# linto-ai/whisper-timestamped

Hardware: NVIDIA H100
Metric: audio-sec/s (RTF) large-v3 1h synthetic @1/2/4/8 H100; DTW GB/s vs HBM peak (higher is better)
Workload: dtype bf16x3 tensor-core GEMMs (float32-accurate), f32 elsewhere, f64 DTW accumulate

## Files before the change

include/wts.h:

```cpp
#ifndef WTS_H
#define WTS_H

#include <stdint.h>

#ifdef __cplusplus
extern "C" {
#endif

#define WTS_VERSION 102
#define WTS_SEG_NONPOSITIVE 1
#define WTS_SEG_PITCH16 2

typedef struct WtsSegDesc {
    int32_t window;
    int32_t row0;
    int32_t last_row;
    int32_t T;
    int32_t f0;
    int32_t F;
    int32_t max_dur;
    int32_t flags;
    int64_t cost_off;
    int64_t jumps_off;
    int64_t dir_off;
// ... 18 lines not shown
int wts_dtw_batch(const void* d_cost, int32_t cost_is_f64,
                  const WtsSegDesc* d_segs, int32_t nseg,
                  uint32_t* d_dir_ws, double* d_bnd_ws,
                  int32_t* d_jumps, int32_t* d_path, const int64_t* d_path_off,
                  int32_t* d_path_len, int32_t* d_status, void* stream);

int wts_dtw_batch_sized(const void* d_cost, int32_t cost_is_f64,
                  const WtsSegDesc* d_segs, int32_t nseg,
                  uint32_t* d_dir_ws, double* d_bnd_ws,
                  int32_t* d_jumps, int32_t* d_path, const int64_t* d_path_off,
                  int32_t* d_path_len, int32_t* d_status, int32_t max_T, int32_t max_F, int32_t all_flags,
                  void* stream);

int wts_disfluency_starts(const float* d_cost, const WtsSegDesc* d_segs, int32_t nseg, const int32_t* d_jumps,
                          int32_t* d_out, void* stream);



typedef struct WtsGemm {
    const void* a;  int64_t lda, a_plane, a_bo, a_bi;
    const void* b;  int64_t ldb, b_plane, b_bo, b_bi;
    int32_t M, N, K, batch_outer, batch_inner;
    float alpha;
    const float* bias;
    int32_t bias_on_m;
    int32_t act;
    const float* residual; int64_t ldr, r_bo, r_bi;
    float* out_f32;   int64_t ldc, c_bo, c_bi;
    void*  out_sb16;  int64_t ldo, o_plane, o_bo, o_bi;
    int32_t head_dim; int64_t head_stride;
    int32_t backend;
    int32_t a_is_f32, b_is_f32;
    const int32_t* row_mask;
} WtsGemm;

int wts_gemm(const WtsGemm* g, void* stream);

int wts_to_sb16(const float* d_x, int64_t n, void* d_hi, void* d_lo, void* stream);

int wts_layernorm(const float* d_x, int64_t ldx, const float* d_gamma, const float* d_beta, int32_t M,
                  int32_t D, void* d_out_sb16, int64_t ldo, int64_t o_plane, float* d_out_f32, int64_t ldf,
                  void* stream);

int wts_softmax_rows(const float* d_s, int64_t lds, int64_t rows, int32_t n, void* d_out_sb16, int64_t ldo,
                     int64_t o_plane, void* stream);

int wts_enc_attention(const void* d_qk, int64_t ld_qk, int64_t qk_plane, const void* d_vt, int64_t ld_vt,
                      int64_t vt_plane, int32_t B, int32_t H, int32_t D, int32_t n_ctx, void* d_out, int64_t ldo,
                      int64_t o_plane, void* stream);

int wts_frames(const float* d_audio, int64_t n_samples, int64_t n_total, int64_t n_frames, void* d_out,
               int64_t o_plane, void* stream);
int wts_power(const float* d_y, int64_t ldy, int64_t n_frames, void* d_out, int64_t ldo, int64_t o_plane,
              void* stream);
int wts_logmel_max(const float* d_m, int64_t n, float* d_max, void* stream);
int wts_logmel_finish(const float* d_m, int64_t n_frames, int32_t n_mels, const float* d_max, float* d_out_f32,
                      void* stream);

int wts_window_gather(const int64_t* d_mel_ptr, int32_t n_mels, const int32_t* d_seek, const int32_t* d_size,
                      int32_t B, void* d_out, int64_t o_plane, void* stream);

int wts_embed(const int32_t* d_tokens, const int32_t* d_positions, const float* d_emb, const float* d_pos,
              int32_t rows, int32_t D, float* d_out, void* stream);

int wts_gather_rows(const float* d_x, int64_t ldx, const int32_t* d_idx, int32_t rows, int32_t D, float* d_out,
                    void* stream);
// ... 84 lines not shown
```

whisper-timestamped_b200/csrc/gemm_tc.cu:

```cuda
#include <cuda_bf16.h>

#include <stdlib.h>

#include "sm90.cuh"

namespace wts {

constexpr int BM = 128, BN = 128, BK = 64;
constexpr int TILE_BYTES = BM * BK * 2;
constexpr int STAGES = 3;
constexpr int STAGE_BYTES = 4 * TILE_BYTES;
constexpr int GT_THREADS = 288;
constexpr int PT_THREADS = 384;
constexpr int PT_PRODUCER_REGS = 40, PT_CONSUMER_REGS = 232;
static_assert(128 * PT_PRODUCER_REGS + 256 * PT_CONSUMER_REGS <= 65536, "setmaxnreg plan exceeds the register file");
constexpr int GROUP_M = 8;
constexpr int GT_SMEM = STAGES * STAGE_BYTES + 256 + 1024;
constexpr int PART_LD = BN + 4;
static_assert(BM * PART_LD * 4 <= STAGES * STAGE_BYTES, "the partial tile lives in the operand ring");

__device__ __forceinline__ float gelu_erf_tc(float v) { return 0.5f * v * (1.0f + erff(v * 0.70710678118654752440f)); }

struct TcArgs {
    WtsGemm g;
    int a_has_bo, a_has_bi, b_has_bo, b_has_bi;
    int split_k;
    int pair_stores;
};

__device__ __forceinline__ int64_t out_offset(const WtsGemm& g, int m, int n, int64_t ld)
{
    return g.head_dim > 0 ? (int64_t)(n / g.head_dim) * g.head_stride + (int64_t)m * ld + (n % g.head_dim)
                          : (int64_t)m * ld + n;
}

__device__ __forceinline__ void store_one(const WtsGemm& g, int m, int n, float t, float* of, __nv_bfloat16* ob)
{
    if (of) of[out_offset(g, m, n, g.ldc)] = t;
    if (ob) {
        const __nv_bfloat16 hi = __float2bfloat16_rn(t);
        __nv_bfloat16* d = ob + out_offset(g, m, n, g.ldo);
        d[0] = hi;
        d[g.o_plane] = __float2bfloat16_rn(t - __bfloat162float(hi));
    }
}

__device__ __forceinline__ float2 pair_values(const WtsGemm& g, int n, bool two, float v0, float v1, float bias_m, const float* res)
{
    float t0 = g.alpha * v0, t1 = g.alpha * v1;
    if (g.bias) {
        t0 += g.bias_on_m ? bias_m : g.bias[n];
        if (two) t1 += g.bias_on_m ? bias_m : g.bias[n + 1];
    }
    if (g.act == 1) { t0 = gelu_erf_tc(t0); t1 = gelu_erf_tc(t1); }
    if (res) { t0 += res[n]; if (two) t1 += res[n + 1]; }
    return make_float2(t0, t1);
}

__device__ __forceinline__ void store_pair_sb16(__nv_bfloat16* dh, int64_t plane, float t0, float t1)
{
// ... 174 lines not shown
            float v[64];
#pragma unroll
            for (int i = 0; i < 64; ++i) v[i] = h ? acc[1][i] : acc[0][i];
            if (pairs) epilogue_frag64<true>(g, tc.zo, tc.zi, tc.m0 + 64 * h + 16 * warp, tc.n0, v);
            else epilogue_frag64<false>(g, tc.zo, tc.zi, tc.m0 + 64 * h + 16 * warp, tc.n0, v);
        }
    }
}

__global__ void __launch_bounds__(GT_THREADS, 1)
gemm_tc_skinny_kernel(const __grid_constant__ CUtensorMap tmA, const __grid_constant__ CUtensorMap tmB, const TcArgs args)
{
    extern __shared__ unsigned char smem_raw[];
    const WtsGemm& g = args.g;
    const uint32_t base = (smem_addr(smem_raw) + 1023u) & ~1023u;
    const uint32_t bar = base + STAGES * STAGE_BYTES;
    const int warp = threadIdx.x >> 5, lane = threadIdx.x & 31;
    const int n0 = blockIdx.x * BN, m0 = blockIdx.y * BM;
    const int S = args.split_k;
    const int z = S > 1 ? 0 : blockIdx.z, zo = z / g.batch_inner, zi = z - zo * g.batch_inner;
    const int nkb_all = (g.K + BK - 1) / BK;
    const int part_k = S > 1 ? blockIdx.z : 0;
    const int kb0 = (int)((int64_t)part_k * nkb_all / S);
    const int nkb = (int)((int64_t)(part_k + 1) * nkb_all / S) - kb0;
    pdl_launch();

    if (threadIdx.x == 256) {
        asm volatile("prefetch.tensormap [%0];" ::"l"(&tmA) : "memory");
        asm volatile("prefetch.tensormap [%0];" ::"l"(&tmB) : "memory");
        for (int s = 0; s < STAGES; ++s) { mbar_init(bar + 8 * s, 1); mbar_init(bar + 32 + 8 * s, 8); }
        asm volatile("fence.mbarrier_init.release.cluster;" ::: "memory");
    }
    __syncthreads();
    pdl_wait();

    float acc[64];
    if (warp == 8) {
        if (lane == 0) {
            const int azo = args.a_has_bo ? zo : 0, azi = args.a_has_bi ? zi : 0;
            const int bzo = args.b_has_bo ? zo : 0, bzi = args.b_has_bi ? zi : 0;
            for (int kb = 0; kb < nkb; ++kb) {
                const int s = kb % STAGES, u = kb / STAGES;
                mbar_wait(bar + 32 + 8 * s, (u & 1) ^ 1);
                const uint32_t full = bar + 8 * s;
                mbar_expect_tx(full, STAGE_BYTES);
                const uint32_t st = base + s * STAGE_BYTES;
                const int kc = (kb0 + kb) * BK;
                tma_load_5d(st, &tmA, full, kc, m0, azi, azo, 0);
                tma_load_5d(st + TILE_BYTES, &tmA, full, kc, m0, azi, azo, 1);
                tma_load_5d(st + 2 * TILE_BYTES, &tmB, full, kc, n0, bzi, bzo, 0);
                tma_load_5d(st + 3 * TILE_BYTES, &tmB, full, kc, n0, bzi, bzo, 1);
            }
        }
    } else {
        const int wg = warp >> 2;
#pragma unroll
        for (int i = 0; i < 64; ++i) acc[i] = 0.f;
        for (int kb = 0; kb < nkb; ++kb) {
            const int s = kb % STAGES, u = kb / STAGES;
            mbar_wait(bar + 8 * s, u & 1);
            const uint32_t st = base + s * STAGE_BYTES;
            const uint64_t a_hi = wg_desc(st + wg * (TILE_BYTES / 2)), a_lo = wg_desc(st + TILE_BYTES + wg * (TILE_BYTES / 2));
            const uint64_t b_hi = wg_desc(st + 2 * TILE_BYTES), b_lo = wg_desc(st + 3 * TILE_BYTES);
            wg_fence();
#pragma unroll
            for (int k = 0; k < BK / 16; ++k) {
                const uint64_t adv = (uint64_t)(k * 2);
                wgmma_ss_n128(acc, a_hi + adv, b_hi + adv, 1);
                wgmma_ss_n128(acc, a_lo + adv, b_hi + adv, 1);
                wgmma_ss_n128(acc, a_hi + adv, b_lo + adv, 1);
            }
            wg_commit();
            wg_wait<1>();
            if (kb > 0 && lane == 0) mbar_arrive(bar + 32 + 8 * ((kb - 1) % STAGES));
        }
        wg_wait<0>();

        const int rl = 64 * wg + 16 * (warp & 3) + (lane >> 2);
        const int cl = 2 * (lane & 3);
        if (S == 1) {
            epilogue_frag64<false>(g, zo, zi, m0 + 64 * wg + 16 * (warp & 3), n0, acc);
        } else {
// ... 76 lines not shown
    }
    return 0;
}

int gemm_tc_launch(const WtsGemm& g, cudaStream_t st)
{
    static int n_sm = 0;
    if (n_sm == 0) {
        WTS_CUDA_CHECK(cudaFuncSetAttribute(gemm_tc_kernel, cudaFuncAttributeMaxDynamicSharedMemorySize, GT_SMEM));
        WTS_CUDA_CHECK(cudaFuncSetAttribute(gemm_tc_skinny_kernel, cudaFuncAttributeMaxDynamicSharedMemorySize, GT_SMEM));
        int dev = 0;
        WTS_CUDA_CHECK(cudaGetDevice(&dev));
        WTS_CUDA_CHECK(cudaDeviceGetAttribute(&n_sm, cudaDevAttrMultiProcessorCount, dev));
    }
    alignas(64) CUtensorMap tmA, tmB;
    int rc = make_map(&tmA, g.a, g.K, g.M, g.lda, g.a_plane, g.batch_inner, g.a_bi, g.batch_outer, g.a_bo, BM, "A");
    if (rc) return rc;
    rc = make_map(&tmB, g.b, g.K, g.N, g.ldb, g.b_plane, g.batch_inner, g.b_bi, g.batch_outer, g.b_bo, BN, "B");
    if (rc) return rc;
    TcArgs args;
    args.g = g;
    args.a_has_bo = g.a_bo != 0; args.a_has_bi = g.a_bi != 0;
    args.b_has_bo = g.b_bo != 0; args.b_has_bi = g.b_bi != 0;
    const int tiles_n = (g.N + BN - 1) / BN, tiles_m = (g.M + BM - 1) / BM, nkb = (g.K + BK - 1) / BK;
    const int batch = g.batch_outer * g.batch_inner;
    cudaLaunchConfig_t cfg = {};
    cfg.dynamicSmemBytes = GT_SMEM;
    cfg.stream = st;
    const bool skinny = tiles_m == 1 && batch == 1 && g.head_dim == 0;
    if (!skinny) {
        const int64_t tiles = (int64_t)tiles_m * tiles_n * batch;
        if (tiles > INT32_MAX / 2) { set_error("wts_gemm(tc): %lld output tiles are too many", (long long)tiles); return -7; }
        args.split_k = 1;
        const bool heads_even = g.head_dim == 0 || (g.head_dim % 2 == 0 && g.head_stride % 2 == 0);
        const bool of_pairs = !g.out_f32 || ((reinterpret_cast<uintptr_t>(g.out_f32) & 7) == 0 && g.ldc % 2 == 0 &&
                                             g.c_bo % 2 == 0 && g.c_bi % 2 == 0);
        const bool ob_pairs = !g.out_sb16 || ((reinterpret_cast<uintptr_t>(g.out_sb16) & 3) == 0 && g.ldo % 2 == 0 &&
                                              g.o_plane % 2 == 0 && g.o_bo % 2 == 0 && g.o_bi % 2 == 0);
        args.pair_stores = !g.row_mask && heads_even && of_pairs && ob_pairs;
        cfg.gridDim = dim3((unsigned)(tiles < n_sm ? tiles : n_sm), 1, 1);
        cfg.blockDim = dim3(PT_THREADS, 1, 1);
        WTS_CUDA_CHECK(cudaLaunchKernelEx(&cfg, gemm_tc_kernel, tmA, tmB, args));
        return 0;
    }
    static const int splitk = []{ const char* e = getenv("WTS_SPLITK"); return e ? atoi(e) : 1; }();
    int split = 1;
    if (splitk && 2 * tiles_n <= n_sm) {
        split = n_sm / tiles_n;
        if (split > 8) split = 8;
        if (split > nkb) split = nkb;
    }
    args.split_k = split;
    args.pair_stores = 0;
    cfg.gridDim = dim3(tiles_n, 1, split);
    cfg.blockDim = dim3(GT_THREADS, 1, 1);
    cudaLaunchAttribute attr[2];
    int na = 0;
    if (split > 1) {
        attr[na].id = cudaLaunchAttributeClusterDimension;
        attr[na].val.clusterDim.x = 1;
        attr[na].val.clusterDim.y = 1;
        attr[na].val.clusterDim.z = split;
        ++na;
    }
    if (pdl_enabled()) {
        attr[na].id = cudaLaunchAttributeProgrammaticStreamSerialization;
        attr[na].val.programmaticStreamSerializationAllowed = 1;
        ++na;
    }
    cfg.attrs = attr;
    cfg.numAttrs = na;
    WTS_CUDA_CHECK(cudaLaunchKernelEx(&cfg, gemm_tc_skinny_kernel, tmA, tmB, args));
    return 0;
}

}
```

whisper-timestamped_b200/csrc/ops.cu:

```cuda
#include "decode_common.cuh"

namespace wts {

__global__ void to_sb16_kernel(const float* __restrict__ x, int64_t n, __nv_bfloat16* __restrict__ hi,
                               __nv_bfloat16* __restrict__ lo)
{
    for (int64_t i = blockIdx.x * (int64_t)blockDim.x + threadIdx.x; i < n; i += (int64_t)gridDim.x * blockDim.x) {
        __nv_bfloat16 h, l;
        split_bf16(x[i], h, l);
        hi[i] = h;
        lo[i] = l;
    }
}

constexpr int LN_THREADS = 128, LN_MAXV = 16;
__global__ void __launch_bounds__(LN_THREADS)
layernorm_kernel(const float* x, int64_t ldx, const float* gamma,
                 const float* beta, int M, int D, __nv_bfloat16* o, int64_t ldo,
                 int64_t o_plane, float* of, int64_t ldf)
{
    pdl_launch();
    pdl_wait();
    __shared__ float red[32];
    const int row = blockIdx.x;
    const float* xr = x + (int64_t)row * ldx;
    float v[LN_MAXV];
    float s = 0.f;
#pragma unroll
    for (int k = 0; k < LN_MAXV; ++k) {
        const int c = threadIdx.x + LN_THREADS * k;
        v[k] = c < D ? xr[c] : 0.f;
        s += v[k];
    }
    const float mean = block_reduce_sum(s, red) / (float)D;
    float q = 0.f;
#pragma unroll
    for (int k = 0; k < LN_MAXV; ++k) {
        const int c = threadIdx.x + LN_THREADS * k;
        const float d = c < D ? v[k] - mean : 0.f;
        q += d * d;
    }
    const float rstd = 1.0f / sqrtf(block_reduce_sum(q, red) / (float)D + 1e-5f);
#pragma unroll
    for (int k = 0; k < LN_MAXV; ++k) {
        const int c = threadIdx.x + LN_THREADS * k;
        if (c < D) {
            const float y = (v[k] - mean) * rstd * gamma[c] + beta[c];
            if (o) {
                __nv_bfloat16 h, l;
                split_bf16(y, h, l);
                o[(int64_t)row * ldo + c] = h;
                o[(int64_t)row * ldo + c + o_plane] = l;
            }
            if (of) of[(int64_t)row * ldf + c] = y;
        }
    }
}

__global__ void __launch_bounds__(128)
softmax_rows_kernel(const float* __restrict__ s, int64_t lds, int64_t rows, int n,
                    __nv_bfloat16* __restrict__ o, int64_t ldo, int64_t o_plane)
{
    const int64_t row = (int64_t)blockIdx.x * 4 + (threadIdx.x >> 5);
    const int lane = threadIdx.x & 31;
    if (row >= rows) return;
    const float* sr = s + row * lds;
    float v[64];
    float mx = -CUDART_INF_F;
#pragma unroll
    for (int k = 0; k < 64; ++k) {
        const int c = lane + 32 * k;
        v[k] = c < n ? sr[c] : -CUDART_INF_F;
        mx = fmaxf(mx, v[k]);
    }
    mx = warp_max(mx);
    float sum = 0.f;
#pragma unroll
    for (int k = 0; k < 64; ++k) {
        v[k] = expf(v[k] - mx);
        sum += v[k];
// ... 324 lines not shown
    float mx = -CUDART_INF_F;
    for (int v = threadIdx.x; v < n; v += blockDim.x) mx = fmaxf(mx, x[v]);
    mx = block_reduce_max(mx, red);
    float s = 0.f;
    for (int v = threadIdx.x; v < n; v += blockDim.x) s += expf(x[v] - mx);
    s = block_reduce_sum(s, red);
    if (threadIdx.x == 0) out[blockIdx.x] = (x[tokens[blockIdx.x]] - mx) - logf(s);
}

}

using namespace wts;

static inline int grid_for(int64_t n, int block, int cap = 132 * 16)
{
    int64_t g = (n + block - 1) / block;
    return (int)(g < 1 ? 1 : (g > cap ? cap : g));
}

extern "C" int wts_to_sb16(const float* d_x, int64_t n, void* d_hi, void* d_lo, void* stream)
{
    if (n <= 0) return 0;
    to_sb16_kernel<<<grid_for(n, 256), 256, 0, (cudaStream_t)stream>>>(d_x, n, (__nv_bfloat16*)d_hi, (__nv_bfloat16*)d_lo);
    WTS_LAUNCH_CHECK();
    return 0;
}

extern "C" int wts_layernorm(const float* d_x, int64_t ldx, const float* d_gamma, const float* d_beta, int32_t M,
                             int32_t D, void* d_out_sb16, int64_t ldo, int64_t o_plane, float* d_out_f32,
                             int64_t ldf, void* stream)
{
    if (M <= 0) return 0;
    if (D > LN_THREADS * LN_MAXV) { set_error("wts_layernorm: D=%d > %d", D, LN_THREADS * LN_MAXV); return -2; }
    WTS_CUDA_CHECK(launch_pdl(layernorm_kernel, dim3(M), dim3(LN_THREADS), 0, (cudaStream_t)stream, d_x, ldx, d_gamma, d_beta, M, D,
                                                                   (__nv_bfloat16*)d_out_sb16, ldo, o_plane, d_out_f32, ldf));
    WTS_LAUNCH_CHECK();
    return 0;
}

extern "C" int wts_softmax_rows(const float* d_s, int64_t lds, int64_t rows, int32_t n, void* d_out_sb16,
                                int64_t ldo, int64_t o_plane, void* stream)
{
    if (rows <= 0) return 0;
    if (n > 2048) { set_error("wts_softmax_rows: n=%d > 2048", n); return -2; }
    softmax_rows_kernel<<<(unsigned)((rows + 3) / 4), 128, 0, (cudaStream_t)stream>>>(d_s, lds, rows, n,
                                                                                     (__nv_bfloat16*)d_out_sb16, ldo, o_plane);
    WTS_LAUNCH_CHECK();
    return 0;
}

extern "C" int wts_frames(const float* d_audio, int64_t n_samples, int64_t n_total, int64_t n_frames, void* d_out,
                          int64_t o_plane, void* stream)
{
    (void)o_plane;
    if (n_frames <= 0) return 0;
    frames_kernel<<<(unsigned)n_frames, 128, 0, (cudaStream_t)stream>>>(d_audio, n_samples, n_total, n_frames, (float*)d_out);
    WTS_LAUNCH_CHECK();
    return 0;
}

extern "C" int wts_power(const float* d_y, int64_t ldy, int64_t n_frames, void* d_out, int64_t ldo, int64_t o_plane,
                         void* stream)
{
    (void)o_plane;
    if (n_frames <= 0) return 0;
    power_kernel<<<(unsigned)((n_frames * 208 + 255) / 256), 256, 0, (cudaStream_t)stream>>>(d_y, ldy, n_frames, (float*)d_out, ldo);
    WTS_LAUNCH_CHECK();
// ... 179 lines not shown
```

whisper-timestamped_b200/csrc/sm90.cuh:

```cuda
#pragma once
#include <cuda.h>
#include <cudaTypedefs.h>

#include <mutex>

#include "common.cuh"

namespace wts {

__device__ __forceinline__ uint32_t smem_addr(const void* p) { return (uint32_t)__cvta_generic_to_shared(p); }

__device__ __forceinline__ void mbar_init(uint32_t bar, uint32_t count)
{
    asm volatile("mbarrier.init.shared::cta.b64 [%0], %1;" ::"r"(bar), "r"(count));
}
__device__ __forceinline__ void mbar_expect_tx(uint32_t bar, uint32_t bytes)
{
    asm volatile("mbarrier.arrive.expect_tx.shared::cta.b64 _, [%0], %1;" ::"r"(bar), "r"(bytes) : "memory");
}
__device__ __forceinline__ void mbar_arrive(uint32_t bar)
{
    asm volatile("mbarrier.arrive.shared::cta.b64 _, [%0];" ::"r"(bar) : "memory");
}
__device__ __forceinline__ void mbar_wait(uint32_t bar, uint32_t parity)
{
    asm volatile(
        "{\n\t"
        ".reg .pred p;\n\t"
        "WAIT_LOOP:\n\t"
        "mbarrier.try_wait.parity.shared::cta.b64 p, [%0], %1;\n\t"
        "@p bra DONE;\n\t"
        "bra WAIT_LOOP;\n\t"
        "DONE:\n\t"
        "}\n" ::"r"(bar), "r"(parity) : "memory");
}
__device__ __forceinline__ void tma_load_4d(uint32_t dst, const CUtensorMap* tm, uint32_t bar, int c0, int c1, int c2, int c3)
{
    asm volatile(
        "cp.async.bulk.tensor.4d.shared::cluster.global.mbarrier::complete_tx::bytes [%0], [%1, {%3, %4, %5, %6}], [%2];"
        ::"r"(dst), "l"(tm), "r"(bar), "r"(c0), "r"(c1), "r"(c2), "r"(c3) : "memory");
}
__device__ __forceinline__ void tma_load_5d(uint32_t dst, const CUtensorMap* tm, uint32_t bar, int c0, int c1, int c2,
                                            int c3, int c4)
{
    asm volatile(
        "cp.async.bulk.tensor.5d.shared::cluster.global.mbarrier::complete_tx::bytes [%0], [%1, {%3, %4, %5, %6, %7}], [%2];"
        ::"r"(dst), "l"(tm), "r"(bar), "r"(c0), "r"(c1), "r"(c2), "r"(c3), "r"(c4) : "memory");
}

__device__ __forceinline__ uint64_t wg_desc(uint32_t saddr)
{
    uint64_t d = 0;
    d |= (uint64_t)((saddr >> 4) & 0x3FFF);
    d |= (uint64_t)1 << 16;
    d |= (uint64_t)(1024 >> 4) << 32;
    d |= (uint64_t)1 << 62;
    return d;
}
__device__ __forceinline__ void wg_fence() { asm volatile("wgmma.fence.sync.aligned;" ::: "memory"); }
__device__ __forceinline__ void wg_commit() { asm volatile("wgmma.commit_group.sync.aligned;" ::: "memory"); }
template <int N> __device__ __forceinline__ void wg_wait() { asm volatile("wgmma.wait_group.sync.aligned %0;" ::"n"(N) : "memory"); }

__device__ __forceinline__ void wgmma_ss_n128(float (&d)[64], uint64_t a, uint64_t b, int scale_d)
{
    asm volatile(
        "{\n\t.reg .pred p;\n\tsetp.ne.b32 p, %66, 0;\n\t"
        "wgmma.mma_async.sync.aligned.m64n128k16.f32.bf16.bf16 {%0, %1, %2, %3, %4, %5, %6, %7, %8, %9, %10, %11, %12, %13, %14, %15, %16, %17, %18, %19, %20, %21, %22, %23, %24, %25, %26, %27, %28, %29, %30, %31, %32, %33, %34, %35, %36, %37, %38, %39, %40, %41, %42, %43, %44, %45, %46, %47, %48, %49, %50, %51, %52, %53, %54, %55, %56, %57, %58, %59, %60, %61, %62, %63}, %64, %65, p, 1, 1, 0, 0;\n\t}\n"
        : "+f"(d[0]), "+f"(d[1]), "+f"(d[2]), "+f"(d[3]), "+f"(d[4]), "+f"(d[5]), "+f"(d[6]), "+f"(d[7]), "+f"(d[8]), "+f"(d[9]), "+f"(d[10]), "+f"(d[11]), "+f"(d[12]), "+f"(d[13]), "+f"(d[14]), "+f"(d[15]), "+f"(d[16]), "+f"(d[17]), "+f"(d[18]), "+f"(d[19]), "+f"(d[20]), "+f"(d[21]), "+f"(d[22]), "+f"(d[23]), "+f"(d[24]), "+f"(d[25]), "+f"(d[26]), "+f"(d[27]), "+f"(d[28]), "+f"(d[29]), "+f"(d[30]), "+f"(d[31]), "+f"(d[32]), "+f"(d[33]), "+f"(d[34]), "+f"(d[35]), "+f"(d[36]), "+f"(d[37]), "+f"(d[38]), "+f"(d[39]), "+f"(d[40]), "+f"(d[41]), "+f"(d[42]), "+f"(d[43]), "+f"(d[44]), "+f"(d[45]), "+f"(d[46]), "+f"(d[47]), "+f"(d[48]), "+f"(d[49]), "+f"(d[50]), "+f"(d[51]), "+f"(d[52]), "+f"(d[53]), "+f"(d[54]), "+f"(d[55]), "+f"(d[56]), "+f"(d[57]), "+f"(d[58]), "+f"(d[59]), "+f"(d[60]), "+f"(d[61]), "+f"(d[62]), "+f"(d[63])
        : "l"(a), "l"(b), "r"(scale_d));
}

__device__ __forceinline__ void wgmma_rs_n64(float (&d)[32], const uint32_t* a, uint64_t b)
{
    asm volatile(
        "{\n\t.reg .pred p;\n\tsetp.ne.b32 p, %37, 0;\n\t"
        "wgmma.mma_async.sync.aligned.m64n64k16.f32.bf16.bf16 {%0, %1, %2, %3, %4, %5, %6, %7, %8, %9, %10, %11, %12, %13, %14, %15, %16, %17, %18, %19, %20, %21, %22, %23, %24, %25, %26, %27, %28, %29, %30, %31}, {%32, %33, %34, %35}, %36, p, 1, 1, 0;\n\t}\n"
        : "+f"(d[0]), "+f"(d[1]), "+f"(d[2]), "+f"(d[3]), "+f"(d[4]), "+f"(d[5]), "+f"(d[6]), "+f"(d[7]), "+f"(d[8]), "+f"(d[9]), "+f"(d[10]), "+f"(d[11]), "+f"(d[12]), "+f"(d[13]), "+f"(d[14]), "+f"(d[15]), "+f"(d[16]), "+f"(d[17]), "+f"(d[18]), "+f"(d[19]), "+f"(d[20]), "+f"(d[21]), "+f"(d[22]), "+f"(d[23]), "+f"(d[24]), "+f"(d[25]), "+f"(d[26]), "+f"(d[27]), "+f"(d[28]), "+f"(d[29]), "+f"(d[30]), "+f"(d[31])
        : "r"(a[0]), "r"(a[1]), "r"(a[2]), "r"(a[3]), "l"(b), "r"(1));
}

// ... 22 lines not shown
```

whisper-timestamped_b200/whisper_timestamped/_native.py:

```python
import ctypes
import os

import numpy as np
import torch

_HERE = os.path.dirname(os.path.abspath(__file__))
LIB_PATH = os.path.join(_HERE, "libwts.so")


class WtsError(RuntimeError):
    pass


class SegDesc(ctypes.Structure):
    _fields_ = [
        ("window", ctypes.c_int32), ("row0", ctypes.c_int32), ("last_row", ctypes.c_int32),
        ("T", ctypes.c_int32), ("f0", ctypes.c_int32), ("F", ctypes.c_int32),
        ("max_dur", ctypes.c_int32), ("flags", ctypes.c_int32),
        ("cost_off", ctypes.c_int64), ("jumps_off", ctypes.c_int64),
        ("dir_off", ctypes.c_int64), ("bnd_off", ctypes.c_int64),
    ]


SEG_DTYPE = np.dtype([
    ("window", "<i4"), ("row0", "<i4"), ("last_row", "<i4"), ("T", "<i4"), ("f0", "<i4"),
    ("F", "<i4"), ("max_dur", "<i4"), ("flags", "<i4"), ("cost_off", "<i8"), ("jumps_off", "<i8"),
    ("dir_off", "<i8"), ("bnd_off", "<i8")])
assert SEG_DTYPE.itemsize == ctypes.sizeof(SegDesc) == 64


class Gemm(ctypes.Structure):
    _fields_ = [
        ("a", ctypes.c_void_p), ("lda", ctypes.c_int64), ("a_plane", ctypes.c_int64), ("a_bo", ctypes.c_int64), ("a_bi", ctypes.c_int64),
        ("b", ctypes.c_void_p), ("ldb", ctypes.c_int64), ("b_plane", ctypes.c_int64), ("b_bo", ctypes.c_int64), ("b_bi", ctypes.c_int64),
        ("M", ctypes.c_int32), ("N", ctypes.c_int32), ("K", ctypes.c_int32), ("batch_outer", ctypes.c_int32), ("batch_inner", ctypes.c_int32),
        ("alpha", ctypes.c_float),
        ("bias", ctypes.c_void_p), ("bias_on_m", ctypes.c_int32), ("act", ctypes.c_int32),
        ("residual", ctypes.c_void_p), ("ldr", ctypes.c_int64), ("r_bo", ctypes.c_int64), ("r_bi", ctypes.c_int64),
        ("out_f32", ctypes.c_void_p), ("ldc", ctypes.c_int64), ("c_bo", ctypes.c_int64), ("c_bi", ctypes.c_int64),
        ("out_sb16", ctypes.c_void_p), ("ldo", ctypes.c_int64), ("o_plane", ctypes.c_int64), ("o_bo", ctypes.c_int64), ("o_bi", ctypes.c_int64),
        ("head_dim", ctypes.c_int32), ("head_stride", ctypes.c_int64),
        ("backend", ctypes.c_int32), ("a_is_f32", ctypes.c_int32), ("b_is_f32", ctypes.c_int32),
        ("row_mask", ctypes.c_void_p),
    ]


class DecodeCfg(ctypes.Structure):
    _fields_ = [("n_vocab", ctypes.c_int32), ("eot", ctypes.c_int32), ("timestamp_begin", ctypes.c_int32),
                ("no_timestamps", ctypes.c_int32), ("max_initial_ts", ctypes.c_int32), ("sample_len", ctypes.c_int32),
                ("n_ctx", ctypes.c_int32), ("tokens_ld", ctypes.c_int32)]


class DecLayer(ctypes.Structure):
    _fields_ = [(n, ctypes.c_void_p) for n in (
        "ln1_g", "ln1_b", "b_qkv", "b_o", "ln2_g", "ln2_b", "b_cq", "b_co", "ln3_g", "ln3_b", "b_fc1", "b_fc2",
        "self_k", "self_v", "cross_k16", "cross_v16", "cross_k_align", "head_slot",
        "sb_qkv", "sb_o", "sb_cq", "sb_co", "sb_fc1", "sb_fc2")] + [(n, ctypes.c_int64) for n in (
        "pl_qkv", "pl_o", "pl_cq", "pl_co", "pl_fc1", "pl_fc2")] + [("align_s0", ctypes.c_int32), ("align_n", ctypes.c_int32)]


class DecodeSteps(ctypes.Structure):
    _fields_ = [(n, ctypes.c_void_p) for n in (
        "layers", "emb", "pos", "ln_g", "ln_b", "tokens", "n_tokens", "n_prompt", "done",
        "logprobs", "full", "last_full", "qk_buf", "suppress", "blank",
        "x", "qkv", "att", "q", "mid", "logits", "emb_sb")] + [("emb_plane", ctypes.c_int64), ("cfg", DecodeCfg)] + [
        (n, ctypes.c_int32) for n in ("n_layer", "D", "H", "n_ctx", "n_audio_ctx", "n_slots", "cap", "lp_ld", "qk_rows",
                                      "max_rows")]


def _load():
    if not os.path.exists(LIB_PATH):
        raise ImportError(
            f"{LIB_PATH} not found: build it with `python whisper-timestamped_b200/build.py` "
            "(the product has no CPU fallback)")
    lib = ctypes.CDLL(LIB_PATH)
    lib.wts_version.restype = ctypes.c_int
# ... 87 lines not shown
```

whisper-timestamped_b200/whisper_timestamped/engine.py:

```python
import ctypes
import os

import numpy as np
import torch

from . import _native as nat
from .alignment import attn_prep, dtw, plan_segments, split_jumps
from .model import SB16
from .windows import N_FRAMES, WindowRecord

N_SAMPLES = 480000
N_CTX_AUDIO = 1500
KPAD = 1504


def _i32(x, dev):
    return torch.as_tensor(np.asarray(x, dtype=np.int32)).to(dev)


class CudaEngine:
    def __init__(self, model, max_batch=None, gemm_backend=None, keep_full_logprobs=False, small_batch_rows=None):
        self.m = model
        self.dev = model.device
        self.w = model.w
# ... 43 lines not shown
        def __enter__(self):
            if self.eng.profile:
                self.a = torch.cuda.Event(enable_timing=True)
                self.b = torch.cuda.Event(enable_timing=True)
                self.a.record(torch.cuda.current_stream(self.eng.dev))

        def __exit__(self, *exc):
            if self.eng.profile:
                self.b.record(torch.cuda.current_stream(self.eng.dev))
                self.eng._events.append((self.name, self.a, self.b))

    def phase(self, name):
        return CudaEngine._Phase(self, name)

    def stage_ms(self, reset=True):
        torch.cuda.synchronize(self.dev)
        out = {}
        self.batch_ms = [(B, steps, self._events[i][1].elapsed_time(self._events[i][2]))
                         for (B, steps, i) in getattr(self, "batch_log", [])]
        self.batch_log = []
        for name, a, b in self._events:
            out[name] = out.get(name, 0.0) + a.elapsed_time(b)
        if reset:
            self._events = []
        return out

    def _st(self):
        return nat.stream_ptr(self.dev)

    def gemm(self, a, b, M, N, K, *, lda=None, ldb=None, a_plane=None, b_plane=None, a_off=0, b_off=0,
             batch=(1, 1), a_b=(0, 0), b_b=(0, 0), alpha=1.0, bias=None, bias_on_m=False, act=0,
             residual=None, ldr=0, r_b=(0, 0), out_f32=None, ldc=0, c_b=(0, 0), c_off=0,
             out_sb=None, ldo=0, o_plane=0, o_b=(0, 0), o_off=0, head_dim=0, head_stride=0,
             a_f32=False, b_f32=False, backend=None, row_mask=None):
        g = nat.Gemm()
        if a_f32:
            g.a, g.lda, g.a_plane = a.data_ptr() + 4 * a_off, lda, 0
        else:
            g.a, g.lda, g.a_plane = a.ptr + 2 * a_off, lda or a.ld, a_plane if a_plane is not None else a.plane
        if b_f32:
            g.b, g.ldb, g.b_plane = b.data_ptr() + 4 * b_off, ldb, 0
        else:
            g.b, g.ldb, g.b_plane = b.ptr + 2 * b_off, ldb or b.ld, b_plane if b_plane is not None else b.plane
        g.a_bo, g.a_bi = a_b
        g.b_bo, g.b_bi = b_b
        g.M, g.N, g.K = M, N, K
        g.batch_outer, g.batch_inner = batch
        g.alpha = alpha
        g.bias = bias.data_ptr() if bias is not None else None
        g.bias_on_m = 1 if bias_on_m else 0
        g.act = act
        if residual is not None:
            g.residual, g.ldr = residual.data_ptr(), ldr
            g.r_bo, g.r_bi = r_b
        if out_f32 is not None:
            g.out_f32, g.ldc = out_f32.data_ptr() + 4 * c_off, ldc
            g.c_bo, g.c_bi = c_b
        if out_sb is not None:
            g.out_sb16, g.ldo, g.o_plane = out_sb.ptr + 2 * o_off, ldo or out_sb.ld, o_plane or out_sb.plane
            g.o_bo, g.o_bi = o_b
        g.head_dim, g.head_stride = head_dim, head_stride
        g.backend = self.backend if backend is None else backend
        g.a_is_f32, g.b_is_f32 = int(a_f32), int(b_f32)
        g.row_mask = row_mask.data_ptr() if row_mask is not None else None
        if a_f32 or b_f32:
            g.backend = 1
        nat.check(nat.lib.wts_gemm(ctypes.byref(g), self._st()), "wts_gemm")
        self.launches += 1

    def layernorm(self, x, gamma, beta, M, D, out_sb=None, out_f32=None):
        nat.check(nat.lib.wts_layernorm(x.data_ptr(), D, gamma.data_ptr(), beta.data_ptr(), M, D,
                                        out_sb.ptr if out_sb is not None else None,
                                        out_sb.ld if out_sb is not None else 0,
                                        out_sb.plane if out_sb is not None else 0,
                                        out_f32.data_ptr() if out_f32 is not None else None, D, self._st()),
                  "wts_layernorm")
        self.launches += 1

    def load_audio(self, audio):
        if isinstance(audio, str):
            import wave
            with wave.open(audio, "rb") as wv:
                if wv.getframerate() != 16000 or wv.getnchannels() != 1 or wv.getsampwidth() != 2:
                    raise RuntimeError("only 16 kHz mono s16 .wav files can be read here (no ffmpeg in this environment)")
                data = wv.readframes(wv.getnframes())
            audio = np.frombuffer(data, np.int16).astype(np.float32) / 32768.0
        if isinstance(audio, np.ndarray):
            audio = torch.from_numpy(np.ascontiguousarray(audio, dtype=np.float32))
        assert isinstance(audio, torch.Tensor), f"Got unexpected audio of type {type(audio)}"
        audio = audio.float()
        if audio.device != self.dev:
            audio = (audio.pin_memory() if audio.device.type == "cpu" else audio).to(self.dev, non_blocking=True)
        return audio.contiguous()

    def log_mel(self, audio, pad_30s=True):
        with self.phase("mel"):
            return self._log_mel(audio, N_SAMPLES if pad_30s else 0)
# ... 55 lines not shown
                      out_sb=vt, ldo=KPAD, o_b=(D * KPAD, 0))
            if fused:
                nat.check(nat.lib.wts_enc_attention(qk.ptr, 2 * D, qk.plane, vt.ptr, KPAD, vt.plane, B, H, D, 1500,
                                                    att.ptr, D, att.plane, st), "wts_enc_attention")
                self.launches += 1
            else:
                self.gemm(qk, qk, 1500, 1500, 64, lda=2 * D, ldb=2 * D, b_off=D, batch=(B, H),
                          a_b=(1500 * 2 * D, 64), b_b=(1500 * 2 * D, 64), out_f32=S, ldc=KPAD,
                          c_b=(H * 1500 * KPAD, 1500 * KPAD))
                nat.check(nat.lib.wts_softmax_rows(S.data_ptr(), KPAD, B * H * 1500, 1500, P.ptr, KPAD, P.plane, st),
                          "wts_softmax_rows")
                self.launches += 1
                self.gemm(P, vt, 1500, 64, 1500, lda=KPAD, ldb=KPAD, batch=(B, H),
                          a_b=(H * 1500 * KPAD, 1500 * KPAD), b_b=(D * KPAD, 64 * KPAD), out_sb=att, ldo=D,
                          o_b=(1500 * D, 64))
            self.gemm(att, a.out, R, D, D, bias=a.out_b, residual=x, ldr=D, out_f32=x, ldc=D)
            self.layernorm(x, blk.mlp_ln_g, blk.mlp_ln_b, R, D, out_sb=hs)
            self.gemm(hs, blk.fc1, R, 4 * D, D, bias=blk.fc1_b, act=1, out_sb=mid)
            self.gemm(mid, blk.fc2, R, D, 4 * D, bias=blk.fc2_b, residual=x, ldr=D, out_f32=x, ldc=D)
        xa = SB16(R, D, dev)
        self.layernorm(x, w.ln_post_g, w.ln_post_b, R, D, out_sb=xa)
        return xa

    def _decoder_rows(self, st8, x, R, row_seq, row_pos, qk_row, qk_buf, active=None):
        d, w, st = self.dims, self.w, self._st()
        D, H, L = d.n_text_state, d.n_text_head, d.n_text_layer
        hs, qkv, att, q, mid = st8["hs"], st8["qkv"], st8["att"], st8["q"], st8["mid"]
        n_slots = len(self.heads)
        for li, blk in enumerate(w.dec):
            a, c = blk.attn, blk.cross
            s0, n_l = self.layer_slots[li]
            kal = st8["ckal"][li]
            self.layernorm(x, a.ln_g, a.ln_b, R, D, out_sb=hs)
            self.gemm(hs, a.qkv, R, 3 * D, D, bias=a.qkv_b, out_f32=qkv, ldc=3 * D, row_mask=active)
            fused_append = active is not None
            if not fused_append:
                nat.check(nat.lib.wts_kv_append(qkv.data_ptr() + 4 * D, qkv.data_ptr() + 8 * D, 3 * D, row_seq.data_ptr(),
                                                row_pos.data_ptr(), R, H, d.n_text_ctx, st8["sk"][li].data_ptr(),
                                                st8["sv"][li].data_ptr(), H * d.n_text_ctx * 64, st), "wts_kv_append")
                self.launches += 1
            nat.check(nat.lib.wts_decoder_attention(2 if fused_append else 0, qkv.data_ptr(), 3 * D, st8["sk"][li].data_ptr(),
                                                    st8["sv"][li].data_ptr(), H * d.n_text_ctx * 64, d.n_text_ctx,
                                                    row_seq.data_ptr(), row_pos.data_ptr(), R, H, att.ptr, att.ld,
                                                    att.plane, None, None, 0, 0, None,
                                                    active.data_ptr() if active is not None else None, st),
                      "wts_decoder_attention")
            self.gemm(att, a.out, R, D, D, bias=a.out_b, residual=x, ldr=D, out_f32=x, ldc=D, row_mask=active)
            self.layernorm(x, c.ln_g, c.ln_b, R, D, out_sb=hs)
            self.gemm(hs, c.q, R, D, D, bias=c.q_b, out_f32=q, ldc=D, row_mask=active)
            nat.check(nat.lib.wts_cross_attention_f16_layer(
                q.data_ptr(), D, st8["ck"][li].data_ptr(), st8["cv"][li].data_ptr(), kal.data_ptr() if kal is not None else None,
                self.head_slot[li].data_ptr(), n_slots, s0, n_l, N_CTX_AUDIO, row_seq.data_ptr(), R, H, att.ptr, att.ld,
                att.plane, qk_buf.data_ptr(), qk_buf.shape[2], qk_row.data_ptr(),
                active.data_ptr() if active is not None else None, st), "wts_cross_attention_f16_layer")
            self.gemm(att, c.out, R, D, D, bias=c.out_b, residual=x, ldr=D, out_f32=x, ldc=D, row_mask=active)
            self.layernorm(x, blk.mlp_ln_g, blk.mlp_ln_b, R, D, out_sb=hs)
            self.gemm(hs, blk.fc1, R, 4 * D, D, bias=blk.fc1_b, act=1, out_sb=mid, row_mask=active)
            self.gemm(mid, blk.fc2, R, D, 4 * D, bias=blk.fc2_b, residual=x, ldr=D, out_f32=x, ldc=D, row_mask=active)
            self.launches += 2

    def _alloc_decoder_state(self, B, R):
        d, dev = self.dims, self.dev
        D, H, L = d.n_text_state, d.n_text_head, d.n_text_layer
        f32 = dict(dtype=torch.float32, device=dev)
        st8 = self._alloc_cross_state(B)
        st8.update(hs=SB16(R, D, dev), att=SB16(R, D, dev), mid=SB16(R, 4 * D, dev),
                   qkv=torch.empty((R, 3 * D), **f32), q=torch.empty((R, D), **f32),
                   sk=[torch.zeros((B, H, d.n_text_ctx, 64), **f32) for _ in range(L)],
                   sv=[torch.zeros((B, H, d.n_text_ctx, 64), **f32) for _ in range(L)])
        return st8

    def _alloc_cross_state(self, B):
        d, dev = self.dims, self.dev
        H, L = d.n_text_head, d.n_text_layer
        return dict(
            ck=[torch.empty((B, H, N_CTX_AUDIO, 64), dtype=torch.float16, device=dev) for _ in range(L)],
            cv=[torch.empty((B, H, N_CTX_AUDIO, 64), dtype=torch.float16, device=dev) for _ in range(L)],
            ckal=[torch.empty((B, n_l, N_CTX_AUDIO, 64), dtype=torch.float32, device=dev) if n_l else None
                  for (_, n_l) in self.layer_slots],
            kvtmp=torch.empty((B, H, N_CTX_AUDIO, 64), dtype=torch.float32, device=dev))

    def _cross_kv(self, xa, st8, B):
        d = self.dims
        D, H = d.n_text_state, d.n_text_head
        for li, blk in enumerate(self.w.dec):
            c = blk.cross
            tmp = st8["kvtmp"]
            s0, n_l = self.layer_slots[li]
            for (wt, bias, dst, al) in ((c.k, None, st8["ck"][li], st8["ckal"][li]), (c.v, c.v_b, st8["cv"][li], None)):
                self.gemm(xa, wt, 1500, D, D, batch=(B, 1), a_b=(1500 * D, 0), bias=bias, out_f32=tmp, ldc=64,
                          c_b=(H * 1500 * 64, 0), head_dim=64, head_stride=1500 * 64)
                nat.check(nat.lib.wts_cross_kv_pack_layer(tmp.data_ptr(), dst.data_ptr(),
                                                          al.data_ptr() if al is not None else None,
                                                          self.head_slot[li].data_ptr(), s0, n_l, B, H, N_CTX_AUDIO,
                                                          self._st()), "wts_cross_kv_pack_layer")
                self.launches += 1

    def _final_logits(self, x_rows, n_rows, logits):
        d, w = self.dims, self.w
        D, V = d.n_text_state, d.n_vocab
        hs = SB16(n_rows, D, self.dev)
        self.layernorm(x_rows, w.ln_g, w.ln_b, n_rows, D, out_sb=hs)
        self.gemm(hs, w.emb_sb, n_rows, V, D, out_f32=logits, ldc=V)

    def decode_windows(self, jobs, setup):
        if getattr(setup, "beam_size", None) is not None or setup.temperature > 0:
            return [self._decode_strategy(job, setup) for job in jobs]
        out = []
        limit = self.batch_limit(setup)
        for i in range(0, len(jobs), limit):
            out.extend(self._decode_batch(jobs[i:i + limit], setup))
        return out

    def window_bytes(self, sample_len):
        d = self.dims
        L, H, D, n_ctx = d.n_text_layer, d.n_text_head, d.n_text_state, d.n_text_ctx
        N, ctx = len(self.heads), N_CTX_AUDIO
        cross = L * H * ctx * 64 * 2 * 2 + N * ctx * 64 * 4 + H * ctx * 64 * 4
        self_kv = 2 * L * H * n_ctx * 64 * 4
        rows = 2 * N * (sample_len + 1) * ctx * 4
        Da = d.n_audio_state
        encoder = 3002 * d.n_mels * 4 + 3001 * Da * 4 + ctx * Da * (4 + 4 + 8 + 4 + 16 + 4) + Da * KPAD * 4
        return cross + self_kv + rows + encoder

    def batch_limit(self, setup):
        key = (tuple(self.heads), setup.sample_len)
        lim = getattr(self, "_limits", {})
        if key not in lim:
            torch.cuda.empty_cache()
            free, _ = torch.cuda.mem_get_info(self.dev)
            ses = getattr(self, "_session", None)
            if ses is not None:
                free += ses["cap"] * self.window_bytes(setup.sample_len)
            lim[key] = max(1, min(self.max_batch, int(0.85 * free) // self.window_bytes(setup.sample_len)))
            self._limits = lim
        return lim[key]
# ... 531 lines not shown
            ses["n_tokens"][:G].fill_(cur)
            self._step_logits(ses)
        ph.__exit__()
        if beam:
            if len(finished) < beam:
                for j in list(np.argsort(sum_lp.numpy()))[::-1]:
                    finished[tuple(seqs[j] + [tok.eot])] = sum_lp[j].item()
                    if len(finished) >= beam:
                        break
            cands = [list(k) for k in finished.keys()]
            cand_lp = list(finished.values())
        else:
            cands = [s_ + [tok.eot] for s_ in seqs]
            cand_lp = sum_lp.tolist()
        cut = []
        for c in cands:
            body = c[P:]
            cut.append(body[:body.index(tok.eot)])
        lp_len = [len(c) for c in cut]
        if setup.length_penalty is None:
            score = [lp / n if n else (float("-inf") if lp < 0 else float("inf")) for lp, n in zip(cand_lp, lp_len)]
        else:
            score = [lp / (((5 + n) / 6) ** setup.length_penalty) for lp, n in zip(cand_lp, lp_len)]
        best = int(np.argmax(score))
        torch.cuda.synchronize(dev)
        return WindowRecord(seek=job["seek"], segment_size=job["segment_size"], prompt=prompt, tokens=cut[best], logprobs=None,
                            ended_by_eot=True, no_speech_prob=float(no_speech.cpu()[0]), qk_window=-1, temperature=T,
                            language=tok.language, sum_logprob=float(cand_lp[best]))

    def _final_logits_static(self, x_rows, n_rows, logits, st8, active=None):
        d, w = self.dims, self.w
        hs = st8["hs_fin"]
        self.layernorm(x_rows, w.ln_g, w.ln_b, n_rows, d.n_text_state, out_sb=hs)
        self.gemm(hs, w.emb_sb, n_rows, d.n_vocab, d.n_text_state, out_f32=logits, ldc=d.n_vocab, row_mask=active)

    @torch.no_grad()
    def teacher_forced(self, mel, tokens_in, i_start, pairs):
        d, dev, st, w = self.dims, self.dev, self._st(), self.w
        tokens_in = [int(t) for t in tokens_in]
        R, D, V = len(tokens_in), d.n_text_state, d.n_vocab
        assert 0 < R <= d.n_text_ctx, f"{R} tokens do not fit the decoder context ({d.n_text_ctx})"
        size = min(N_FRAMES, int(mel.shape[0]))
        with self.phase("encoder"):
            xa = self.encode([dict(mel=mel, seek=0, segment_size=size)])
        st8 = getattr(self, "_tf_state", None)
        if st8 is None:
            st8 = self._tf_state = self._alloc_decoder_state(1, d.n_text_ctx)
        with self.phase("cross_kv"):
            self._cross_kv(xa, st8, 1)
        del xa
        rows = R - (i_start - 1)
        qk_buf = torch.zeros((1, len(self.heads), rows, N_CTX_AUDIO), dtype=torch.float32, device=dev)
        row_seq = _i32([0] * R, dev)
        row_pos = _i32(list(range(R)), dev)
        row_tok = _i32(tokens_in, dev)
        qk_row = _i32([p - (i_start - 1) if p >= i_start - 1 else -1 for p in range(R)], dev)
        x = torch.empty((R, D), dtype=torch.float32, device=dev)
        with self.phase("prefill"):
            nat.check(nat.lib.wts_embed(row_tok.data_ptr(), row_pos.data_ptr(), w.emb.data_ptr(), w.dec_pos.data_ptr(), R, D,
                                        x.data_ptr(), st), "wts_embed")
            self.launches += 1
            self._decoder_rows(st8, x, R, row_seq, row_pos, qk_row, qk_buf)
            vals = np.zeros(0, dtype=np.float32)
            if pairs:
                steps = sorted({int(s_) for (s_, _) in pairs})
                index = {s_: i for i, s_ in enumerate(steps)}
                sel = _i32(steps, dev)
# ... 83 lines not shown
```

Baseline: 622.6.

## Issue constant weight loads and L2 prefetches before PDL wait in decoder GEMMs

For GEMMs whose B operand is a constant weight, the skinny (split-K/decode) path now issues the first pipeline stages' B-tile TMA loads and L2 prefetches for the following k-blocks before the programmatic-dependent-launch wait. This lets weight loads overlap the tail of the previous kernel. Layernorm similarly loads gamma and beta into registers before the PDL wait when there are few rows. The risk is extra register pressure in layernorm and relying on correct expect_tx accounting across the split barrier arrivals.

```diff
diff --git a/include/wts.h b/include/wts.h
--- a/include/wts.h
+++ b/include/wts.h
@@ -74,6 +74,7 @@
     int32_t backend;
     int32_t a_is_f32, b_is_f32;
     const int32_t* row_mask;
+    int32_t b_const;
 } WtsGemm;
 
 int wts_gemm(const WtsGemm* g, void* stream);
diff --git a/whisper-timestamped_b200/csrc/gemm_tc.cu b/whisper-timestamped_b200/csrc/gemm_tc.cu
--- a/whisper-timestamped_b200/csrc/gemm_tc.cu
+++ b/whisper-timestamped_b200/csrc/gemm_tc.cu
@@ -10,6 +10,7 @@
 constexpr int TILE_BYTES = BM * BK * 2;
 constexpr int STAGES = 3;
 constexpr int STAGE_BYTES = 4 * TILE_BYTES;
+constexpr int EARLY_L2_KB = 8;
 constexpr int GT_THREADS = 288;
 constexpr int PT_THREADS = 384;
 constexpr int PT_PRODUCER_REGS = 40, PT_CONSUMER_REGS = 232;
@@ -26,6 +27,7 @@
     int a_has_bo, a_has_bi, b_has_bo, b_has_bi;
     int split_k;
     int pair_stores;
+    int early_b;
 };
 
 __device__ __forceinline__ int64_t out_offset(const WtsGemm& g, int m, int n, int64_t ld)
@@ -266,22 +268,38 @@
         asm volatile("fence.mbarrier_init.release.cluster;" ::: "memory");
     }
     __syncthreads();
+    const int azo = args.a_has_bo ? zo : 0, azi = args.a_has_bi ? zi : 0;
+    const int bzo = args.b_has_bo ? zo : 0, bzi = args.b_has_bi ? zi : 0;
+    int early = 0;
+    if (threadIdx.x == 256 && args.early_b) {
+        early = min(nkb, STAGES);
+        for (int kb = 0; kb < early; ++kb) {
+            const uint32_t full = bar + 8 * kb, st = base + kb * STAGE_BYTES;
+            mbar_expect_tx_only(full, 2 * TILE_BYTES);
+            tma_load_5d(st + 2 * TILE_BYTES, &tmB, full, (kb0 + kb) * BK, n0, bzi, bzo, 0);
+            tma_load_5d(st + 3 * TILE_BYTES, &tmB, full, (kb0 + kb) * BK, n0, bzi, bzo, 1);
+        }
+        for (int kb = early; kb < min(nkb, STAGES + EARLY_L2_KB); ++kb) {
+            tma_prefetch_5d(&tmB, (kb0 + kb) * BK, n0, bzi, bzo, 0);
+            tma_prefetch_5d(&tmB, (kb0 + kb) * BK, n0, bzi, bzo, 1);
+        }
+    }
     pdl_wait();
 
     float acc[64];
     if (warp == 8) {
         if (lane == 0) {
-            const int azo = args.a_has_bo ? zo : 0, azi = args.a_has_bi ? zi : 0;
-            const int bzo = args.b_has_bo ? zo : 0, bzi = args.b_has_bi ? zi : 0;
             for (int kb = 0; kb < nkb; ++kb) {
                 const int s = kb % STAGES, u = kb / STAGES;
                 mbar_wait(bar + 32 + 8 * s, (u & 1) ^ 1);
                 const uint32_t full = bar + 8 * s;
-                mbar_expect_tx(full, STAGE_BYTES);
+                const bool b_sent = kb < early;
+                mbar_expect_tx(full, b_sent ? 2 * TILE_BYTES : STAGE_BYTES);
                 const uint32_t st = base + s * STAGE_BYTES;
                 const int kc = (kb0 + kb) * BK;
                 tma_load_5d(st, &tmA, full, kc, m0, azi, azo, 0);
                 tma_load_5d(st + TILE_BYTES, &tmA, full, kc, m0, azi, azo, 1);
+                if (b_sent) continue;
                 tma_load_5d(st + 2 * TILE_BYTES, &tmB, full, kc, n0, bzi, bzo, 0);
                 tma_load_5d(st + 3 * TILE_BYTES, &tmB, full, kc, n0, bzi, bzo, 1);
             }
@@ -424,6 +442,7 @@
         const int64_t tiles = (int64_t)tiles_m * tiles_n * batch;
         if (tiles > INT32_MAX / 2) { set_error("wts_gemm(tc): %lld output tiles are too many", (long long)tiles); return -7; }
         args.split_k = 1;
+        args.early_b = 0;
         const bool heads_even = g.head_dim == 0 || (g.head_dim % 2 == 0 && g.head_stride % 2 == 0);
         const bool of_pairs = !g.out_f32 || ((reinterpret_cast<uintptr_t>(g.out_f32) & 7) == 0 && g.ldc % 2 == 0 &&
                                              g.c_bo % 2 == 0 && g.c_bi % 2 == 0);
@@ -435,6 +454,8 @@
         WTS_CUDA_CHECK(cudaLaunchKernelEx(&cfg, gemm_tc_kernel, tmA, tmB, args));
         return 0;
     }
+    const char* early_env = getenv("WTS_GEMM_EARLY_B");
+    args.early_b = g.b_const && !(early_env && atoi(early_env) == 0);
     static const int splitk = []{ const char* e = getenv("WTS_SPLITK"); return e ? atoi(e) : 1; }();
     int split = 1;
     if (splitk && 2 * tiles_n <= n_sm) {
diff --git a/whisper-timestamped_b200/csrc/ops.cu b/whisper-timestamped_b200/csrc/ops.cu
--- a/whisper-timestamped_b200/csrc/ops.cu
+++ b/whisper-timestamped_b200/csrc/ops.cu
@@ -13,13 +13,23 @@
     }
 }
 
-constexpr int LN_THREADS = 128, LN_MAXV = 16;
+constexpr int LN_THREADS = 128, LN_MAXV = 16, LN_EARLY_ROWS = 1024;
+template <bool EARLY_PARAMS>
 __global__ void __launch_bounds__(LN_THREADS)
 layernorm_kernel(const float* x, int64_t ldx, const float* gamma,
                  const float* beta, int M, int D, __nv_bfloat16* o, int64_t ldo,
                  int64_t o_plane, float* of, int64_t ldf)
 {
     pdl_launch();
+    float gm[EARLY_PARAMS ? LN_MAXV : 1], bt[EARLY_PARAMS ? LN_MAXV : 1];
+    if (EARLY_PARAMS) {
+#pragma unroll
+        for (int k = 0; k < LN_MAXV; ++k) {
+            const int c = threadIdx.x + LN_THREADS * k;
+            gm[k] = c < D ? gamma[c] : 0.f;
+            bt[k] = c < D ? beta[c] : 0.f;
+        }
+    }
     pdl_wait();
     __shared__ float red[32];
     const int row = blockIdx.x;
@@ -45,7 +55,7 @@
     for (int k = 0; k < LN_MAXV; ++k) {
         const int c = threadIdx.x + LN_THREADS * k;
         if (c < D) {
-            const float y = (v[k] - mean) * rstd * gamma[c] + beta[c];
+            const float y = (v[k] - mean) * rstd * (EARLY_PARAMS ? gm[k] : gamma[c]) + (EARLY_PARAMS ? bt[k] : beta[c]);
             if (o) {
                 __nv_bfloat16 h, l;
                 split_bf16(y, h, l);
@@ -436,7 +446,7 @@
 {
     if (M <= 0) return 0;
     if (D > LN_THREADS * LN_MAXV) { set_error("wts_layernorm: D=%d > %d", D, LN_THREADS * LN_MAXV); return -2; }
-    WTS_CUDA_CHECK(launch_pdl(layernorm_kernel, dim3(M), dim3(LN_THREADS), 0, (cudaStream_t)stream, d_x, ldx, d_gamma, d_beta, M, D,
+    WTS_CUDA_CHECK(launch_pdl(M <= LN_EARLY_ROWS ? layernorm_kernel<true> : layernorm_kernel<false>, dim3(M), dim3(LN_THREADS), 0, (cudaStream_t)stream, d_x, ldx, d_gamma, d_beta, M, D,
                                                                    (__nv_bfloat16*)d_out_sb16, ldo, o_plane, d_out_f32, ldf));
     WTS_LAUNCH_CHECK();
     return 0;
diff --git a/whisper-timestamped_b200/csrc/sm90.cuh b/whisper-timestamped_b200/csrc/sm90.cuh
--- a/whisper-timestamped_b200/csrc/sm90.cuh
+++ b/whisper-timestamped_b200/csrc/sm90.cuh
@@ -17,6 +17,10 @@
 __device__ __forceinline__ void mbar_expect_tx(uint32_t bar, uint32_t bytes)
 {
     asm volatile("mbarrier.arrive.expect_tx.shared::cta.b64 _, [%0], %1;" ::"r"(bar), "r"(bytes) : "memory");
+}
+__device__ __forceinline__ void mbar_expect_tx_only(uint32_t bar, uint32_t bytes)
+{
+    asm volatile("mbarrier.expect_tx.shared::cta.b64 [%0], %1;" ::"r"(bar), "r"(bytes) : "memory");
 }
 __device__ __forceinline__ void mbar_arrive(uint32_t bar)
 {
@@ -46,6 +50,11 @@
     asm volatile(
         "cp.async.bulk.tensor.5d.shared::cluster.global.mbarrier::complete_tx::bytes [%0], [%1, {%3, %4, %5, %6, %7}], [%2];"
         ::"r"(dst), "l"(tm), "r"(bar), "r"(c0), "r"(c1), "r"(c2), "r"(c3), "r"(c4) : "memory");
+}
+__device__ __forceinline__ void tma_prefetch_5d(const CUtensorMap* tm, int c0, int c1, int c2, int c3, int c4)
+{
+    asm volatile("cp.async.bulk.prefetch.tensor.5d.L2.global.tile [%0, {%1, %2, %3, %4, %5}];"
+                 ::"l"(tm), "r"(c0), "r"(c1), "r"(c2), "r"(c3), "r"(c4) : "memory");
 }
 
 __device__ __forceinline__ uint64_t wg_desc(uint32_t saddr)
diff --git a/whisper-timestamped_b200/whisper_timestamped/_native.py b/whisper-timestamped_b200/whisper_timestamped/_native.py
--- a/whisper-timestamped_b200/whisper_timestamped/_native.py
+++ b/whisper-timestamped_b200/whisper_timestamped/_native.py
@@ -41,7 +41,7 @@
         ("out_sb16", ctypes.c_void_p), ("ldo", ctypes.c_int64), ("o_plane", ctypes.c_int64), ("o_bo", ctypes.c_int64), ("o_bi", ctypes.c_int64),
         ("head_dim", ctypes.c_int32), ("head_stride", ctypes.c_int64),
         ("backend", ctypes.c_int32), ("a_is_f32", ctypes.c_int32), ("b_is_f32", ctypes.c_int32),
-        ("row_mask", ctypes.c_void_p),
+        ("row_mask", ctypes.c_void_p), ("b_const", ctypes.c_int32),
     ]
 
 
diff --git a/whisper-timestamped_b200/whisper_timestamped/engine.py b/whisper-timestamped_b200/whisper_timestamped/engine.py
--- a/whisper-timestamped_b200/whisper_timestamped/engine.py
+++ b/whisper-timestamped_b200/whisper_timestamped/engine.py
@@ -99,7 +99,7 @@
              batch=(1, 1), a_b=(0, 0), b_b=(0, 0), alpha=1.0, bias=None, bias_on_m=False, act=0,
              residual=None, ldr=0, r_b=(0, 0), out_f32=None, ldc=0, c_b=(0, 0), c_off=0,
              out_sb=None, ldo=0, o_plane=0, o_b=(0, 0), o_off=0, head_dim=0, head_stride=0,
-             a_f32=False, b_f32=False, backend=None, row_mask=None):
+             a_f32=False, b_f32=False, backend=None, row_mask=None, b_const=False):
         g = nat.Gemm()
         if a_f32:
             g.a, g.lda, g.a_plane = a.data_ptr() + 4 * a_off, lda, 0
@@ -130,6 +130,7 @@
         g.backend = self.backend if backend is None else backend
         g.a_is_f32, g.b_is_f32 = int(a_f32), int(b_f32)
         g.row_mask = row_mask.data_ptr() if row_mask is not None else None
+        g.b_const = int(b_const)
         if a_f32 or b_f32:
             g.backend = 1
         nat.check(nat.lib.wts_gemm(ctypes.byref(g), self._st()), "wts_gemm")
@@ -251,7 +252,8 @@
             s0, n_l = self.layer_slots[li]
             kal = st8["ckal"][li]
             self.layernorm(x, a.ln_g, a.ln_b, R, D, out_sb=hs)
-            self.gemm(hs, a.qkv, R, 3 * D, D, bias=a.qkv_b, out_f32=qkv, ldc=3 * D, row_mask=active)
+            self.gemm(hs, a.qkv, R, 3 * D, D, bias=a.qkv_b, out_f32=qkv, ldc=3 * D, row_mask=active,
+                      b_const=True)
             fused_append = active is not None
             if not fused_append:
                 nat.check(nat.lib.wts_kv_append(qkv.data_ptr() + 4 * D, qkv.data_ptr() + 8 * D, 3 * D, row_seq.data_ptr(),
@@ -264,18 +266,23 @@
                                                     att.plane, None, None, 0, 0, None,
                                                     active.data_ptr() if active is not None else None, st),
                       "wts_decoder_attention")
-            self.gemm(att, a.out, R, D, D, bias=a.out_b, residual=x, ldr=D, out_f32=x, ldc=D, row_mask=active)
+            self.gemm(att, a.out, R, D, D, bias=a.out_b, residual=x, ldr=D, out_f32=x, ldc=D, row_mask=active,
+                      b_const=True)
             self.layernorm(x, c.ln_g, c.ln_b, R, D, out_sb=hs)
-            self.gemm(hs, c.q, R, D, D, bias=c.q_b, out_f32=q, ldc=D, row_mask=active)
+            self.gemm(hs, c.q, R, D, D, bias=c.q_b, out_f32=q, ldc=D, row_mask=active,
+                      b_const=True)
             nat.check(nat.lib.wts_cross_attention_f16_layer(
                 q.data_ptr(), D, st8["ck"][li].data_ptr(), st8["cv"][li].data_ptr(), kal.data_ptr() if kal is not None else None,
                 self.head_slot[li].data_ptr(), n_slots, s0, n_l, N_CTX_AUDIO, row_seq.data_ptr(), R, H, att.ptr, att.ld,
                 att.plane, qk_buf.data_ptr(), qk_buf.shape[2], qk_row.data_ptr(),
                 active.data_ptr() if active is not None else None, st), "wts_cross_attention_f16_layer")
-            self.gemm(att, c.out, R, D, D, bias=c.out_b, residual=x, ldr=D, out_f32=x, ldc=D, row_mask=active)
+            self.gemm(att, c.out, R, D, D, bias=c.out_b, residual=x, ldr=D, out_f32=x, ldc=D, row_mask=active,
+                      b_const=True)
             self.layernorm(x, blk.mlp_ln_g, blk.mlp_ln_b, R, D, out_sb=hs)
-            self.gemm(hs, blk.fc1, R, 4 * D, D, bias=blk.fc1_b, act=1, out_sb=mid, row_mask=active)
-            self.gemm(mid, blk.fc2, R, D, 4 * D, bias=blk.fc2_b, residual=x, ldr=D, out_f32=x, ldc=D, row_mask=active)
+            self.gemm(hs, blk.fc1, R, 4 * D, D, bias=blk.fc1_b, act=1, out_sb=mid, row_mask=active,
+                      b_const=True)
+            self.gemm(mid, blk.fc2, R, D, 4 * D, bias=blk.fc2_b, residual=x, ldr=D, out_f32=x, ldc=D, row_mask=active,
+                      b_const=True)
             self.launches += 2
 
     def _alloc_decoder_state(self, B, R):
@@ -320,7 +327,7 @@
         D, V = d.n_text_state, d.n_vocab
         hs = SB16(n_rows, D, self.dev)
         self.layernorm(x_rows, w.ln_g, w.ln_b, n_rows, D, out_sb=hs)
-        self.gemm(hs, w.emb_sb, n_rows, V, D, out_f32=logits, ldc=V)
+        self.gemm(hs, w.emb_sb, n_rows, V, D, out_f32=logits, ldc=V, b_const=True)
 
     def decode_windows(self, jobs, setup):
         if getattr(setup, "beam_size", None) is not None or setup.temperature > 0:
@@ -918,7 +925,8 @@
         d, w = self.dims, self.w
         hs = st8["hs_fin"]
         self.layernorm(x_rows, w.ln_g, w.ln_b, n_rows, d.n_text_state, out_sb=hs)
-        self.gemm(hs, w.emb_sb, n_rows, d.n_vocab, d.n_text_state, out_f32=logits, ldc=d.n_vocab, row_mask=active)
+        self.gemm(hs, w.emb_sb, n_rows, d.n_vocab, d.n_text_state, out_f32=logits, ldc=d.n_vocab, row_mask=active,
+                      b_const=True)
 
     @torch.no_grad()
     def teacher_forced(self, mel, tokens_in, i_start, pairs):
```

New measurement: 639.7, median of 6. +2.7%, better.
